# liangfu/dspnet

Measured on AMD Instinct MI355X. Metric: training images/sec at 512x512 multitask, higher is better.
Workload: dtype f32; 1 GPU; resnet-50 multitask (det+depth+seg) 512x512, 8 det classes, 19 seg classes, N=6132 anchors, forward+backward+SGD; batch_per_gpu=32, global_batch=32, parallelism=dp1, f16x2_fallback_calls=0

## Files before the change

### dspnet_amd/csrc/conv.hip

```cpp
#include "dspn_common.h"
#include "bn_final_job.h"
#include "dspn_store.h"
#include "dspn_pieces.h"
#include "conv_geom.h"
#include <cstdlib>
#include "../../include/dspn_nn.h"

using dspn::st_t;
using dspn::kHalf;
using dspn::u32x4_t;

namespace {

using dspn::conv::f32x16;
using dspn::conv::bf16x8;
using dspn::pieces::bf16x4;
typedef __attribute__((address_space(3))) bf16x4 lds_bf16x4;

constexpr int kLdsRowH = kHalf ? 72 : 40;
__device__ __forceinline__ bf16x4 to_bf16x4(const float4 v) {
  bf16x4 r = {(__bf16)v.x, (__bf16)v.y, (__bf16)v.z, (__bf16)v.w};
  return r;
}

// ... 1579 lines not shown
  if (cfg64 >= 0 && Cout > 32 && Cout <= 64 && tiles(kNtBm[cfg64], kNtBn[cfg64]) >= min_tiles) cfg = cfg64;
  if ((g_debug_bits >> 8) & 7) cfg = ((g_debug_bits >> 8) & 7) - 1;
  return cfg;
}
int output_absmax_pass(const st_t *out, const ConvGeom &g, hipStream_t s) {
#ifndef DSPN_HALF
  if (g.bn_dy_absmax && !g.bn_sums) {
    if (!(g.dense && g.obs == (long long)g.Hg * g.Wg * g.ldc && g.ldc % 4 == 0))
      return dspn::fail(DSPN_ERR_ARG_, "conv2d_forward: the output magnitude block needs a dense output with ldc %% 4 == 0");
    return dspn_absmax_f32(out, (long long)g.N * g.Hg * g.Wg, g.ldc, nullptr, nullptr, 0, reinterpret_cast<float *>(g.bn_dy_absmax), s);
  }
#endif
  return 0;
}
int dispatch_nt(const st_t *in, const st_t *w, const float *bias, st_t *out, const ConvGeom &g_in,
                hipStream_t s, SplitWs ws, const st_t *residual = nullptr) {
  ConvGeom g = g_in;
  g.dbg = g_debug_bits;
  constexpr uintptr_t amask = 4 * sizeof(st_t) - 1;
  if (g.ldc % 4 == 0 && g.obs % 4 == 0 && (reinterpret_cast<uintptr_t>(out) & amask) == 0 &&
      (!residual || (reinterpret_cast<uintptr_t>(residual) & amask) == 0))
    g.flags |= 16;
  {
    const long long ib = (long long)sizeof(st_t) * g.N * g.Hin * g.Win * g.Cin,
                    wb = (long long)sizeof(st_t) * g.Cout * g.WTAPS * g.Cin;
    if (ib >= (1ll << 31) || wb >= (1ll << 31))
      return dspn::fail(DSPN_ERR_ARG_, "conv: tensors of 2 GiB or more are not supported by the buffer-addressed kernel");
    g.in_bytes = (unsigned)ib; g.w_bytes = (unsigned)wb;
  }
  const long long M = (long long)g.N * g.Hg * g.Wg;
  if (M <= 0) return output_absmax_pass(out, g, s);
  const bool pre = !kHalf && g.bf16 >= 2 && ((g.Cin / kEPC) & 7) == 0;
  if (pre) {
    if (!g.w_planes)
      return dspn::fail(DSPN_ERR_ARG_, "conv: the split math modes with a multiple of 32 input channels (%d) need the weight operand as piece planes (dspn_conv2d_weight_planes_f32)", g.Cin);
    w = static_cast<const st_t *>(g.w_planes);
    g.w_bytes = (unsigned)((g.bf16 == 3 ? 4ll : 6ll) * g.Cout * g.WTAPS * g.Cin);
  }
  const int cfg = nt_config(M, g.Cout);
  const long long nblk = ((M + kNtBm[cfg] - 1) / kNtBm[cfg]) * ((g.Cout + kNtBn[cfg] - 1) / kNtBn[cfg]);
  const int nk = (g.TR * g.TS * (g.Cin / kEPC) + 7) >> 3;
  int splits = 1, per = nk;
  if (g.a_planes && !(pre && g.bf16 == 3 && !g.in_scale))
    return dspn::fail(DSPN_ERR_ARG_, "conv: a piece-plane operand needs DSPN_MATH_F32_F16X2, a multiple of 32 channels (%d) and no input affine", g.Cin);
  if (g.stats && (!g.dense || !(g.flags & 16) || g.Cout % 4 != 0))
    return dspn::fail(DSPN_ERR_ARG_, "conv2d_forward: output statistics need a dense, 16-byte aligned output with Cout %% 4 == 0");
  if (g.bn_sums && (g.in_scale || g.stats))
    return dspn::fail(DSPN_ERR_ARG_, "conv: BatchNorm-backward sums cannot be combined with an input affine or output statistics");
  if (g.bn_sums && (!(g.flags & 16) || g.Cout % 4 != 0))
    return dspn::fail(DSPN_ERR_ARG_, "conv2d_dgrad: BatchNorm sums need a 16-byte aligned dx with Cin %% 4 == 0");
  if (g.dense && nblk < 192 && nk >= 16 && ws.ptr && !g.stats && !g.bn_sums) {
    splits = (int)std::min<long long>((384 + nblk - 1) / nblk, nk / 8);
    splits = std::max(1, std::min(splits, 32));
    while (splits > 1 && sizeof(float) * (size_t)splits * M * g.Cout > ws.bytes) --splits;
    per = (nk + splits - 1) / splits;
    splits = (nk + per - 1) / per;
  }
  static const int eight_mode = (int)dspn::env_int("DSPN_NT_8WAVE", -1);
  const bool one_tap = g.TR * g.TS == 1;
  const bool eight = eight_mode == 0 ? false : eight_mode == 1 ? true : (kHalf || g.bf16 >= 2) ? true
                     : ((!g.stats && !g.bn_sums) || (eight_mode == 2 && one_tap && g.bn_sums) || (eight_mode == 3 && one_tap));
  bool wide_ok = splits == 1 && (cfg == 0 || (cfg == 2 && g.Cout > 32 && g.Cout <= 64)) && (g.flags & 16) && g.Cout % 4 == 0 &&
                 g.TR * g.TS > 0;
  if (kHalf) wide_ok = wide_ok && !g.in_scale && g.Cin % 64 == 0 && dspn::wide_tiles_mode() >= 2;
  else wide_ok = wide_ok && pre && g.bf16 == 3;
  if (const dspn::conv::WideRoute route = wide_ok ? dspn::conv::wide_route(g, M, nk) : dspn::conv::WideRoute{})
    return dspn::conv::launch_wide(route, in, w, bias, out, g, s, residual);
  const int rc = cfg == 0 && eight ? launch_nt<4, 2, 1, 2>(in, w, bias, out, g, s, splits, per, ws.ptr, residual)
                 : cfg == 0        ? launch_nt<2, 2, 2, 2>(in, w, bias, out, g, s, splits, per, ws.ptr, residual)
                 : cfg == 1        ? launch_nt<2, 2, 2, 1>(in, w, bias, out, g, s, splits, per, ws.ptr, residual)
                 : cfg == 2        ? launch_nt<2, 2, 1, 1>(in, w, bias, out, g, s, splits, per, ws.ptr, residual)
                                   : launch_nt<4, 1, 2, 1>(in, w, bias, out, g, s, splits, per, ws.ptr, residual);
  return rc ? rc : output_absmax_pass(out, g, s);
}

struct WgradPlan { int bm; int bn; int splits; int pps; };
constexpr int kPlanPK = 64;
static_assert(kPlanPK % kPK == 0, "split sizes must be whole k-steps");
long long wgrad_x_footprint(long long P, int Cin, int taps, int stride) { return taps > 1 ? 4ll * P * Cin * std::min(stride, 2) * std::min(stride, 2) : 0; }
WgradPlan wgrad_plan(long long P, int Cout, int J, long long x_bytes = 0, long long max_splits = 1 << 30) {
  WgradPlan p;
  p.bm = Cout <= 32 ? 32 : (Cout <= 64 ? 64 : 128);
  if (p.bm == 128 && (Cout + 63) / 64 * 64 < (Cout + 127) / 128 * 128) p.bm = 64;
  p.bn = (J <= 64 && p.bm == 128) ? 64 : 128;
  if (const char *e = getenv("DSPN_WG_TILE")) {
    const int t = atoi(e);
    p.bm = t == 0 ? 32 : (t == 1 ? 64 : 128);
    p.bn = t == 2 ? 64 : 128;
  }
  const long long tiles = (long long)((Cout + p.bm - 1) / p.bm) * ((J + p.bn - 1) / p.bn);
  const long long lds = 4ll * std::max(2 * kPK * (p.bm + p.bn), p.bm * (p.bn + 4));
  const long long slots = 256 * std::min<long long>(8, (160ll << 10) / lds);
  long long s_min = 1;
  if (x_bytes > 0) s_min = (x_bytes + (32ll << 20) - 1) / (32ll << 20);
  const long long s_max = std::max<long long>(1, std::min<long long>(std::min<long long>(P / 128, 1024), max_splits));
  s_min = std::min(s_min, s_max);
  const double flop_per_pix = 2.0 * p.bm * p.bn, slot_rate = 120e12 / (double)slots, ovh_pix = 160;
  double best = 1e30;
  long long splits = s_min;
  for (long long sp = s_min; sp <= s_max; ++sp) {
    const long long pps = ((P + sp - 1) / sp + kPlanPK - 1) / kPlanPK * kPlanPK;
    const long long real = (P + pps - 1) / pps;
    const long long rounds = (tiles * real + slots - 1) / slots;
    const double t = (double)rounds * ((double)pps + ovh_pix) * flop_per_pix / slot_rate +
                     (double)real * Cout * J * 8.0 / 4e12;
    if (t < best * 0.999) { best = t; splits = sp; }
    if (tiles * sp > 8 * slots) break;
  }
  if (const char *e = getenv("DSPN_WG_SPLITS")) splits = std::max<long long>(1, std::min<long long>(atoll(e), s_max));
  splits = std::min(splits, s_max);
  long long pps = ((P + splits - 1) / splits + kPlanPK - 1) / kPlanPK * kPlanPK;
  p.splits = (int)((P + pps - 1) / pps);
  p.pps = (int)pps;
  return p;
}

struct WgradLaunch { const st_t *x, *dy; float *slab; const WgradGeom &g; int kt, jt, rows; size_t lds; hipStream_t s; };
template <int WM, int WN, int TM, int TN, int MODE, bool INTF>
int launch_wgrad_impl(const WgradLaunch &a) {
  auto kern = conv_wgrad_kernel<WM, WN, TM, TN, MODE, INTF>;
  static dspn::KernelDeviceState st;
  if (const int dev = dspn::ensure_dynamic_lds(reinterpret_cast<const void *>(kern), a.lds, st, "conv_wgrad"); dev < 0) return dev;
  hipLaunchKernelGGL(kern, dim3(a.kt * a.jt, a.rows), dim3(WM * WN * 64), a.lds, a.s, a.x, a.dy, a.slab, a.g, a.kt, a.jt);
  return 0;
}
template <int WM, int WN, int TM, int TN, int MODE>
int launch_wgrad_mode(const WgradLaunch &a) {
  return a.g.in_scale ? launch_wgrad_impl<WM, WN, TM, TN, MODE, true>(a) : launch_wgrad_impl<WM, WN, TM, TN, MODE, false>(a);
}
template <int WM, int WN, int TM, int TN>
int launch_wgrad_tile(const WgradLaunch &a) {
  switch (kHalf ? 1 : a.g.bf16 != 3 ? a.g.bf16 : a.g.x_planes ? 5 + a.g.dy_planes : 3 + a.g.dy_planes) {
#ifndef DSPN_HALF
    case 6: return launch_wgrad_impl<WM, WN, TM, TN, 6, false>(a);
    case 5: return launch_wgrad_impl<WM, WN, TM, TN, 5, false>(a);
    case 4: return launch_wgrad_mode<WM, WN, TM, TN, 4>(a);
    case 3: return launch_wgrad_mode<WM, WN, TM, TN, 3>(a);
    case 2: return launch_wgrad_mode<WM, WN, TM, TN, 2>(a);
    case 0: return launch_wgrad_mode<WM, WN, TM, TN, 0>(a);
#endif
    default: return launch_wgrad_mode<WM, WN, TM, TN, 1>(a);
  }
}
static int launch_wgrad(int BM, int BN, const WgradLaunch &a) {
#ifndef DSPN_HALF
  static const bool wgw_env = dspn::env_int("DSPN_WGW", 1) != 0;
  if (a.g.bf16 == 3 && a.g.x_planes && a.g.dy_planes && BM == 128 && BN == 128 && wgw_env && dspn::wide_tiles_mode() != 1) {
    auto kern = conv_wgw_kernel<2, 2, 2>;
    const size_t lds_w = std::max<size_t>(2 * (size_t)kPK * (128 + 128) * 4, sizeof(float) * 128 * (128 + 4));
    static dspn::KernelDeviceState st;
    if (const int dev = dspn::ensure_dynamic_lds(reinterpret_cast<const void *>(kern), lds_w, st, "conv_wgrad (wide)"); dev < 0) return dev;
    hipLaunchKernelGGL(kern, dim3(a.kt * a.jt, a.rows), dim3(256), lds_w, a.s, a.x, a.dy, a.slab, a.g, a.kt, a.jt);
    return 0;
  }
#endif
  if (BM == 32) return launch_wgrad_tile<1, 4, 1, 1>(a);
  if (BM == 64) return launch_wgrad_tile<2, 2, 1, 2>(a);
  if (BN == 64) return launch_wgrad_tile<2, 2, 2, 1>(a);
  return launch_wgrad_tile<4, 2, 1, 2>(a);
}

}

extern "C" {

#ifdef DSPN_ABLATE
#ifdef DSPN_HALF
int dspn_debug_set_bf16(int bits) { g_debug_bits = bits; return 0; }
#else
int dspn_debug_set(int bits) { g_debug_bits = bits; return 0; }
int dspn_debug_read_stamps(unsigned *host, int words, int clear) {
  if (hipMemcpyFromSymbol(host, HIP_SYMBOL(g_phase_stamps), sizeof(unsigned) * (size_t)std::min(words, 8192 * 8)) != hipSuccess) return 1;
  if (clear) { static unsigned z[8192 * 8]; (void)hipMemcpyToSymbol(HIP_SYMBOL(g_phase_stamps), z, sizeof(z)); }
  return 0;
}
#endif
#endif

#ifndef DSPN_HALF
size_t dspn_conv2d_split_workspace_bytes(long long out_pixels, int Cout) {
  if (out_pixels <= 0 || Cout <= 0) return 0;
  const long long capped = std::min<long long>(out_pixels * Cout, 192ll * 64 * 64 * 4);
  return sizeof(float) * 32 * (size_t)capped;
}
#endif

static int split_math(int *math, int plane_bits) {
  const int flags = *math & (DSPN_MATH_UNSCALED_OK | plane_bits);
  *math &= ~flags;
  return flags;
}
static int check_math_mode(const char *who, int math) {
  DSPN_REQUIRE(math >= DSPN_MATH_FP32 && math <= DSPN_MATH_F32_F16X2, "%s: math is one of DSPN_MATH_*", who);
  return 0;
}
static int check_math_blocks(const char *who, int math, int flags, const float *a_absmax, const float *b_absmax) {
  DSPN_REQUIRE(dspn::kHalf || math != DSPN_MATH_F32_F16X2 || (flags & DSPN_MATH_UNSCALED_OK) || (a_absmax && b_absmax),
               "%s: DSPN_MATH_F32_F16X2 needs the magnitude block of both operands (dspn_absmax_f32); a caller who knows that every |operand| < 65504 passes math | DSPN_MATH_UNSCALED_OK", who);
  return 0;
}
struct InAffine { const float *scale, *shift; int relu; };
struct OpScales { const float *a, *b; int a_planes = 0; };

static int conv2d_forward_one(int math, OpScales scales, const st_t *x, InAffine tf, float *stats, float *minmax, const st_t *w, const void *w_planes, const float *bias, const st_t *residual, st_t *y, int N,
                            int H, int W, int Cin, int Cout, int R, int S, int stride, int pad_h, int pad_w,
                            int dil, int Ho, int Wo, long long y_batch_stride, int y_ldc,
                            int relu, int accumulate, void *workspace, size_t workspace_bytes,
                            void *stream) {
  DSPN_REQUIRE(x && (w || w_planes) && y, "conv2d_forward: null pointer");
  DSPN_REQUIRE(Cin % kEPC == 0, "conv2d_forward: Cin must be a multiple of %d (pad channels), got %d", kEPC, Cin);
  DSPN_REQUIRE(N > 0 && H > 0 && W > 0 && Cout > 0 && R > 0 && S > 0 && stride > 0 && dil > 0,
               "conv2d_forward: bad geometry");
  DSPN_REQUIRE(Ho == (H + 2 * pad_h - dil * (R - 1) - 1) / stride + 1 &&
                   Wo == (W + 2 * pad_w - dil * (S - 1) - 1) / stride + 1,
               "conv2d_forward: output size mismatch");
  ConvGeom g;
  memset(&g, 0, sizeof(g));
  g.N = N; g.Hin = H; g.Win = W; g.Cin = Cin; g.Hg = Ho; g.Wg = Wo;
  g.ish = stride; g.isw = stride; g.ioh = -pad_h; g.iow = -pad_w; g.idh = dil; g.idw = dil;
  g.TR = R; g.TS = S; g.WTAPS = R * S; g.WS = S; g.wr0 = 0; g.wrs = 1; g.ws0 = 0; g.wss = 1;
  g.Cout = Cout;
  g.ldc = y_ldc > 0 ? y_ldc : Cout;
  g.obs = y_batch_stride > 0 ? y_batch_stride : (long long)Ho * Wo * g.ldc;
  g.OW = Wo; g.osh = 1; g.osw = 1; g.ooh = 0; g.oow = 0;
  g.dense = (g.obs == (long long)Ho * Wo * g.ldc);
  g.flags = (bias ? 1 : 0) | (relu ? 2 : 0) | (accumulate ? 4 : 0) | (residual ? 8 : 0) | ((tf.scale && tf.relu) ? 32 : 0);
  g.in_scale = tf.scale; g.in_shift = tf.shift;
  g.stats = stats;
  g.minmax = (stats && !kHalf && math == DSPN_MATH_F32_F16X2) ? minmax : nullptr;
  g.bn_dy_absmax = (!stats && minmax && !kHalf && math == DSPN_MATH_F32_F16X2) ? reinterpret_cast<unsigned *>(minmax) : nullptr;
  g.bf16 = kHalf ? 1 : math;
  g.w_planes = w_planes;
  g.a_absmax = scales.a; g.b_absmax = scales.b;
  g.a_planes = scales.a_planes;
#ifndef DSPN_HALF
  if (math == DSPN_MATH_F32_F16X2 && R == 7 && S == 7 && stride == 2 && pad_h == 3 && pad_w == 3 && dil == 1 && Cin == 4 &&
      Cout == 64 && !bias && !relu && !accumulate && !residual && !tf.scale && g.dense && g.ldc == Cout && scales.a && scales.b &&
      !scales.a_planes && (reinterpret_cast<uintptr_t>(x) & 15) == 0 &&
      !g.bn_dy_absmax && (!stats || kNtBm[nt_config((long long)N * Ho * Wo, Cout)] == 64)) {
    const int rc = dspn::conv::launch_stem(x, w, y, N, H, W, Cin, Cout, Ho, Wo, scales.a, scales.b, stats, g.minmax, (hipStream_t)stream);
    if (rc <= 0) return rc;
  }
#endif
  return dispatch_nt(x, w, bias, y, g, (hipStream_t)stream,
                     SplitWs{static_cast<float *>(workspace), workspace ? workspace_bytes : 0}, residual);
}

static int batch_chunk(int N, long long bytes_per_image) {
  const long long lim = (1ll << 31) - 1;
  if (bytes_per_image <= 0 || N * bytes_per_image <= lim) return N;
  return (int)std::max<long long>(1, lim / bytes_per_image);
}

static int stats_layout(long long out_pixels, int Cout, int *tile_rows) {
  if (out_pixels <= 0 || Cout <= 0 || Cout % 4 != 0) return 0;
  const int bm = kNtBm[nt_config(out_pixels, Cout)];
  if (tile_rows) *tile_rows = bm;
  return (int)((out_pixels + bm - 1) / bm);
}
#ifndef DSPN_HALF
int dspn_conv2d_stats_layout(long long out_pixels, int Cout, int *tile_rows) { return stats_layout(out_pixels, Cout, tile_rows); }
#endif

int DSPN_FN(dspn_conv2d_forward_bn)(const st_t *x, const float *in_scale, const float *in_shift, int in_relu,
                               const st_t *w, const void *w_planes, const float *bias, const st_t *residual, st_t *y, int N,
                               int H, int W, int Cin, int Cout, int R, int S, int stride, int pad_h, int pad_w,
                               int dil, int Ho, int Wo, long long y_batch_stride, int y_ldc,
                               int relu, int accumulate, float *out_stats, size_t out_stats_bytes, float *out_minmax,
                               int math, const float *x_absmax, const float *w_absmax,
                               void *workspace, size_t workspace_bytes, void *stream) {
  DSPN_REQUIRE(N > 0 && H > 0 && W > 0 && Cin > 0, "conv2d_forward: bad geometry");
  const int flags = split_math(&math, DSPN_MATH_X_PLANES), x_planes = (flags & DSPN_MATH_X_PLANES) ? 1 : 0;
  if (const int rc = check_math_mode("conv2d_forward", math)) return rc;
  DSPN_REQUIRE(!x_planes || (!dspn::kHalf && math == DSPN_MATH_F32_F16X2 && Cin % 32 == 0 && x_absmax && !in_scale),
               "conv2d_forward: DSPN_MATH_X_PLANES needs DSPN_MATH_F32_F16X2, Cin %% 32 == 0, no input affine and the block the planes were cut by (x_absmax)");
  if (const int rc = check_math_blocks("conv2d_forward", math, flags, x_absmax, w_absmax)) return rc;
  DSPN_REQUIRE((in_scale == nullptr) == (in_shift == nullptr), "conv2d_forward: in_scale and in_shift go together");
  if (out_stats) {
    int tile_rows = 0;
    const int mt = stats_layout((long long)N * Ho * Wo, Cout, &tile_rows);
    DSPN_REQUIRE(mt > 0 && out_stats_bytes >= sizeof(float) * 2 * (size_t)mt * Cout,
                 "conv2d_forward: out_stats needs dspn_conv2d_stats_layout() tiles x 2 x Cout floats and Cout %% 4 == 0");
    DSPN_REQUIRE(batch_chunk(N, (long long)sizeof(st_t) * H * W * Cin) == N, "conv2d_forward: out_stats is not available for inputs of 2 GiB or more");
  }
  const int ldc = y_ldc > 0 ? y_ldc : Cout;
  const long long ybs = y_batch_stride > 0 ? y_batch_stride : (long long)Ho * Wo * ldc;
  const int nb = batch_chunk(N, (long long)sizeof(st_t) * H * W * Cin);
  for (int n0 = 0; n0 < N; n0 += nb) {
    const int n = std::min(nb, N - n0);
    const int rc = conv2d_forward_one(math, OpScales{x_absmax, w_absmax, x_planes}, x + (long long)n0 * H * W * Cin, InAffine{in_scale, in_shift, in_relu}, out_stats, out_minmax, w, w_planes, bias,
                                      residual ? residual + (long long)n0 * ybs : nullptr, y + (long long)n0 * ybs, n, H, W,
                                      Cin, Cout, R, S, stride, pad_h, pad_w, dil, Ho, Wo, y_batch_stride, y_ldc, relu,
                                      accumulate, workspace, workspace_bytes, stream);
    if (rc) return rc;
  }
  return 0;
}

#ifndef DSPN_HALF
int dspn_conv2d_forward_f32(const float *x, const float *w, const float *bias, const float *residual, float *y, int N,
                            int H, int W, int Cin, int Cout, int R, int S, int stride, int pad_h, int pad_w,
                            int dil, int Ho, int Wo, long long y_batch_stride, int y_ldc,
                            int relu, int accumulate, void *workspace, size_t workspace_bytes,
                            void *stream) {
  return dspn_conv2d_forward_bn_f32(x, nullptr, nullptr, 0, w, nullptr, bias, residual, y, N, H, W, Cin, Cout, R, S, stride, pad_h,
                                    pad_w, dil, Ho, Wo, y_batch_stride, y_ldc, relu, accumulate, nullptr, 0, nullptr,
// ... 380 lines not shown
```

### dspnet_amd/csrc/conv_geom.h

```cpp
#pragma once
#include <hip/hip_runtime.h>

namespace dspn {
namespace conv {

typedef float f32x16 __attribute__((ext_vector_type(16)));
typedef __bf16 bf16x8 __attribute__((ext_vector_type(8)));

template <typename st_t>
struct ConvGeomT {
  int N, Hin, Win, Cin;
  int Hg, Wg;
  int ish, isw, ioh, iow, idh, idw;
  int TR, TS;
  int WTAPS, WS, wr0, wrs, ws0, wss;
  int Cout;
  long long obs;
  int OW, osh, osw, ooh, oow, ldc;
  int flags;
  int dense;
  int dbg;
  int bf16;
  unsigned in_bytes, w_bytes;
  const float *in_scale, *in_shift;
  float *stats;
  float *minmax;
  const st_t *bn_x;
  const float *bn_scale, *bn_shift, *bn_mean, *bn_rstd;
  float *bn_sums;
  int bn_relu, bn_tile_base;
  unsigned *bn_dy_absmax;
  const float *a_absmax, *b_absmax;
  int a_planes;
  const void *w_planes;
};

__device__ __forceinline__ int xcd_remap(int bid, int nblk) {
  const int q = nblk >> 3, r = nblk & 7, x = bid & 7;
  const int start = x < r ? x * (q + 1) : r * (q + 1) + (x - r) * q;
  return start + (bid >> 3);
}


enum class WideTile { None, P256x128, P128x256, P128x128, P256x64, F128x256, F128x128, F256x64 };
enum class WideLoop { Plain, Spanning, Direct };
struct WideRoute {
  WideTile tile = WideTile::None; WideLoop loop = WideLoop::Plain;
  explicit operator bool() const { return tile != WideTile::None; }
};
WideRoute wide_route(const ConvGeomT<float> &g, long long M, int nk);
WideRoute wide_route(const ConvGeomT<__bf16> &g, long long M, int nk);
int launch_wide(WideRoute r, const float *in, const float *w_planes, const float *bias, float *out, const ConvGeomT<float> &g,
                hipStream_t s, const float *residual);
int launch_wide(WideRoute r, const __bf16 *in, const __bf16 *w, const float *bias, __bf16 *out, const ConvGeomT<__bf16> &g,
                hipStream_t s, const __bf16 *residual);

int launch_stem(const float *x, const float *w, float *y, int N, int H, int W, int Cin, int Cout, int Ho, int Wo,
                const float *x_absmax, const float *w_absmax, float *stats, float *minmax, hipStream_t s);

}
}
```

### dspnet_amd/csrc/conv_stem.h

```cpp

constexpr int kStemSeg = 256;
constexpr int kStemRing = 9;
constexpr int kStemRowPx = 2 * kStemSeg + 8;
constexpr int kStemRowBytes = kStemRowPx * 8;
constexpr int kStemWRow = 7 * 2 * 64 + 16;
constexpr int kStemWBytes = 64 * kStemWRow;

__global__ __launch_bounds__(512, 2) void conv_stem_f16x2_kernel(
    const float *__restrict__ x, const float *__restrict__ w, float *__restrict__ y, int N, int H, int W, int Ho, int Wo,
    int rows_per_strip, const float *__restrict__ x_absmax, const float *__restrict__ w_absmax,
    float *__restrict__ stats, float *__restrict__ minmax) {
  extern __shared__ __attribute__((aligned(1024))) char ssm[];
  char *sW = ssm;
  char *sX = ssm + kStemWBytes;
  float *sRed = reinterpret_cast<float *>(sX + kStemRing * 2 * kStemRowBytes);
  const int tid = threadIdx.x, lane = tid & 63, wave = tid >> 6;
  const float sc_a = operand_scale(x_absmax), sc_b = operand_scale(w_absmax);
  const float inv_a = 1.f / sc_a, inv_b = 1.f / sc_b;
  const int segs = Wo / kStemSeg, strips = (Ho + rows_per_strip - 1) / rows_per_strip;
  int b = blockIdx.x;
  const int seg = b % segs; b /= segs;
  const int strip = b % strips;
  const int n = b / strips;
  const int oy0 = strip * rows_per_strip, oy1 = min(Ho, oy0 + rows_per_strip);
  const int ix0 = 2 * seg * kStemSeg - 3;

  for (int i = tid; i < 64 * 7 * 8; i += 512) {
    const int s = i & 7, r = (i >> 3) % 7, k = i / 56;
    float4 v = make_float4(0.f, 0.f, 0.f, 0.f);
    if (s < 7) v = *reinterpret_cast<const float4 *>(w + ((k * 7 + r) * 7 + s) * 4);
    bf16x4 p0, p1;
    split2h(v, sc_b, p0, p1);
    repair_inf(p0, p1);
    *reinterpret_cast<bf16x4 *>(sW + k * kStemWRow + (r * 2 + 0) * 64 + s * 8) = p0;
    *reinterpret_cast<bf16x4 *>(sW + k * kStemWRow + (r * 2 + 1) * 64 + s * 8) = p1;
  }
  const float4 *xin = reinterpret_cast<const float4 *>(x) + (long long)n * H * W;
  auto load_px = [&](const int iy, const int p) __attribute__((always_inline)) {
    const int ix = ix0 + p;
    float4 v = make_float4(0.f, 0.f, 0.f, 0.f);
    if (p < kStemRowPx && (unsigned)iy < (unsigned)H && (unsigned)ix < (unsigned)W) v = xin[(long long)iy * W + ix];
    return v;
  };
  auto store_px = [&](const int slot, const int p, const float4 v) __attribute__((always_inline)) {
    if (p >= kStemRowPx) return;
    bf16x4 p0, p1;
    split2h(v, sc_a, p0, p1);
    *reinterpret_cast<bf16x4 *>(sX + (slot * 2 + 0) * kStemRowBytes + p * 8) = p0;
    *reinterpret_cast<bf16x4 *>(sX + (slot * 2 + 1) * kStemRowBytes + p * 8) = p1;
  };
  const int iy_base = 2 * oy0 - 3;
  for (int j = 0; j < 7; ++j) {
    store_px(j, tid, load_px(iy_base + j, tid));
    store_px(j, tid + 512, load_px(iy_base + j, tid + 512));
  }
  __syncthreads();

  const int frow = lane & 31, half = lane >> 5;
  const int px = wave * 32 + frow;
  f32x16 acc[2];
  for (int oy = oy0; oy < oy1; ++oy) {
    const int j0 = ((oy - oy0) * 2) % kStemRing;
    const int iy_new = 2 * oy + 4;
    float4 n0 = load_px(iy_new, tid), n1 = load_px(iy_new, tid + 512), n2 = load_px(iy_new + 1, tid), n3 = load_px(iy_new + 1, tid + 512);
#pragma unroll
    for (int r = 0; r < 16; ++r) { acc[0][r] = 0.f; acc[1][r] = 0.f; }
#pragma unroll
    for (int r = 0; r < 7; ++r) {
      int slot = j0 + r; slot = slot >= kStemRing ? slot - kStemRing : slot;
      const char *xa = sX + slot * 2 * kStemRowBytes + (2 * px + 2 * half) * 8;
      const char *wb = sW + frow * kStemWRow + r * 128 + half * 16;
#pragma unroll
      for (int kk = 0; kk < 2; ++kk) {
        const bf16x8 a0 = *reinterpret_cast<const bf16x8 *>(xa + kk * 32), a1 = *reinterpret_cast<const bf16x8 *>(xa + kStemRowBytes + kk * 32);
        bf16x8 b0[2], b1[2];
#pragma unroll
        for (int j = 0; j < 2; ++j) {
          b0[j] = *reinterpret_cast<const bf16x8 *>(wb + j * (32 * kStemWRow) + kk * 32);
          b1[j] = *reinterpret_cast<const bf16x8 *>(wb + j * (32 * kStemWRow) + 64 + kk * 32);
        }
#pragma unroll
        for (int j = 0; j < 2; ++j) {
          acc[j] = __builtin_amdgcn_mfma_f32_32x32x16_f16(__builtin_bit_cast(f16x8, a1), __builtin_bit_cast(f16x8, b0[j]), acc[j], 0, 0, 0);
          acc[j] = __builtin_amdgcn_mfma_f32_32x32x16_f16(__builtin_bit_cast(f16x8, a0), __builtin_bit_cast(f16x8, b1[j]), acc[j], 0, 0, 0);
          acc[j] = __builtin_amdgcn_mfma_f32_32x32x16_f16(__builtin_bit_cast(f16x8, a0), __builtin_bit_cast(f16x8, b0[j]), acc[j], 0, 0, 0);
        }
      }
    }
    const long long m_row = ((long long)n * Ho + oy) * Wo + seg * kStemSeg + wave * 32;
    float s1[2], mn[2], mx[2];
#pragma unroll
    for (int j = 0; j < 2; ++j) {
      const int co = j * 32 + frow;
      s1[j] = 0.f; mn[j] = __builtin_huge_valf(); mx[j] = -__builtin_huge_valf();
#pragma unroll
      for (int q = 0; q < 16; ++q) {
        const float v = acc[j][q] * inv_a * inv_b;
        acc[j][q] = v;
        y[(m_row + (q & 3) + 8 * (q >> 2) + 4 * half) * 64 + co] = v;
        s1[j] += v; mn[j] = fminf(mn[j], v); mx[j] = fmaxf(mx[j], v);
      }
    }
    if (stats) {
#pragma unroll
      for (int j = 0; j < 2; ++j) {
        const float mean16 = s1[j] * (1.f / 16.f);
        float m2 = 0.f;
#pragma unroll
        for (int q = 0; q < 16; ++q) { const float d = acc[j][q] - mean16; m2 += d * d; }
        const float mean_o = __shfl_xor(mean16, 32, 64), m2_o = __shfl_xor(m2, 32, 64);
        const float d = mean_o - mean16;
        const float mean32 = mean16 + 0.5f * d;
        const float m2_32 = m2 + m2_o + d * d * 8.f;
        const float mn32 = fminf(mn[j], __shfl_xor(mn[j], 32, 64)), mx32 = fmaxf(mx[j], __shfl_xor(mx[j], 32, 64));
        if (half == 0) *reinterpret_cast<float4 *>(sRed + (wave * 64 + j * 32 + frow) * 4) = make_float4(mean32, m2_32, mn32, mx32);
      }
    }
    __syncthreads();
    if (stats && tid < 256) {
      const int tl = tid >> 6, co = tid & 63;
      const float4 a = *reinterpret_cast<const float4 *>(sRed + ((2 * tl) * 64 + co) * 4);
      const float4 c = *reinterpret_cast<const float4 *>(sRed + ((2 * tl + 1) * 64 + co) * 4);
      const float d = c.x - a.x;
      const long long t = (((long long)n * Ho + oy) * Wo + seg * kStemSeg) / 64 + tl;
      stats[(t * 2 + 0) * 64 + co] = a.x + 0.5f * d;
      stats[(t * 2 + 1) * 64 + co] = a.y + c.y + d * d * 16.f;
      if (minmax) {
        minmax[(t * 2 + 0) * 64 + co] = fminf(a.z, c.z);
        minmax[(t * 2 + 1) * 64 + co] = fmaxf(a.w, c.w);
      }
    }
    int sl0 = j0 + 7; sl0 = sl0 >= kStemRing ? sl0 - kStemRing : sl0;
    int sl1 = j0 + 8; sl1 = sl1 >= kStemRing ? sl1 - kStemRing : sl1;
    store_px(sl0, tid, n0); store_px(sl0, tid + 512, n1);
    store_px(sl1, tid, n2); store_px(sl1, tid + 512, n3);
    __syncthreads();
  }
}

int launch_conv_stem(const float *x, const float *w, float *y, int N, int H, int W, int Cin, int Cout, int Ho, int Wo,
                     const float *x_absmax, const float *w_absmax, float *stats, float *minmax, hipStream_t s) {
  if (dspn::wide_tiles_mode() == 1) return 1;
  if (Cin != 4 || Cout != 64 || Wo % kStemSeg != 0 || Ho != (H + 6 - 7) / 2 + 1 || Wo != (W + 6 - 7) / 2 + 1) return 1;
  const int lds = kStemWBytes + kStemRing * 2 * kStemRowBytes + 8 * 64 * 4 * (int)sizeof(float);
  static dspn::KernelDeviceState st;
  if (const int dev = dspn::ensure_dynamic_lds(reinterpret_cast<const void *>(conv_stem_f16x2_kernel), (size_t)lds, st, "conv_stem"); dev < 0) return dev;
  int rows = 16;
  while (rows > 8 && (long long)N * ((Ho + rows - 1) / rows) * (Wo / kStemSeg) < 512) rows -= 4;
  const long long grid = (long long)N * ((Ho + rows - 1) / rows) * (Wo / kStemSeg);
  {
    dspn::ProfScope prof(0, s);
    hipLaunchKernelGGL(conv_stem_f16x2_kernel, dim3((unsigned)grid), dim3(512), lds, s, x, w, y, N, H, W, Ho, Wo, rows, x_absmax,
                       w_absmax, stats, minmax);
  }
  return dspn::check_launch("conv_stem");
}
```

### dspnet_amd/csrc/conv_wide.hip

```cpp
#include "dspn_common.h"
#include "dspn_store.h"
#include "dspn_pieces.h"
#include "conv_geom.h"
#include "../../include/dspn_nn.h"
#include <algorithm>
#include <type_traits>

namespace {
using namespace dspn::pieces;
using dspn::st_t;
using dspn::kHalf;
using dspn::u32x4_t;
using dspn::conv::f32x16;
using dspn::conv::bf16x8;
using dspn::conv::xcd_remap;
using dspn::conv::WideLoop;
using ConvGeom = dspn::conv::ConvGeomT<st_t>;
#include "conv_wide.h"
#ifndef DSPN_HALF
#include "conv_stem.h"
#endif
}

#ifndef DSPN_HALF
namespace {
struct AbsminRowsDesc { const float *w; unsigned *out; int rows, row_len; long long begin; };
__global__ __launch_bounds__(256) void absmin_rows_batch_kernel(const AbsminRowsDesc *__restrict__ d, int n) {
  __shared__ float sm[4];
  const long long row = blockIdx.x;
  int lo = 0, hi = n - 1;
  while (lo < hi) {
    const int mid = (lo + hi + 1) >> 1;
    if (d[mid].begin <= row) lo = mid; else hi = mid - 1;
  }
  const AbsminRowsDesc e = d[lo];
  const float *p = e.w + (row - e.begin) * (long long)e.row_len;
  float m = 0.f;
  for (int i = threadIdx.x; i < e.row_len; i += 256) m = fmaxf(m, fabsf(p[i]));
#pragma unroll
  for (int o = 32; o >= 1; o >>= 1) m = fmaxf(m, __shfl_xor(m, o, 64));
  if ((threadIdx.x & 63) == 0) sm[threadIdx.x >> 6] = m;
  __syncthreads();
  if (threadIdx.x == 0) {
    m = fmaxf(fmaxf(sm[0], sm[1]), fmaxf(sm[2], sm[3]));
    if (m > 0.f && m < __builtin_huge_valf()) atomicMin(e.out, __float_as_uint(m));
  }
}
__global__ __launch_bounds__(256) void tile_minmax_kernel(const float4 *__restrict__ x, long long rows, int C4, int tile_rows,
                                                          float4 *__restrict__ minmax) {
  const long long t = blockIdx.x;
  const long long r0 = t * tile_rows, r1 = r0 + tile_rows < rows ? r0 + tile_rows : rows;
  for (int c = blockIdx.y * 256 + threadIdx.x; c < C4; c += gridDim.y * 256) {
    constexpr float kInf = __builtin_huge_valf();
    float4 mn = make_float4(kInf, kInf, kInf, kInf), mx = make_float4(-kInf, -kInf, -kInf, -kInf);
    for (long long r = r0; r < r1; ++r) {
      const float4 v = x[r * C4 + c];
      mn.x = fminf(mn.x, v.x); mn.y = fminf(mn.y, v.y); mn.z = fminf(mn.z, v.z); mn.w = fminf(mn.w, v.w);
      mx.x = fmaxf(mx.x, v.x); mx.y = fmaxf(mx.y, v.y); mx.z = fmaxf(mx.z, v.z); mx.w = fmaxf(mx.w, v.w);
    }
    minmax[(t * 2 + 0) * C4 + c] = mn;
    minmax[(t * 2 + 1) * C4 + c] = mx;
  }
}
}

extern "C" {
int dspn_absmin_rows_batch_f32(const void *table, int n, long long total_rows, void *stream) {
  DSPN_REQUIRE(table && n > 0 && total_rows > 0 && total_rows < (1ll << 31), "absmin_rows_batch: bad argument");
  static_assert(sizeof(AbsminRowsDesc) == 32, "table row layout: 2 pointers, 2 ints, 1 int64");
  hipLaunchKernelGGL(absmin_rows_batch_kernel, dim3((unsigned)total_rows), dim3(256), 0, (hipStream_t)stream,
                     static_cast<const AbsminRowsDesc *>(table), n);
  return dspn::check_launch("absmin_rows_batch");
}
int dspn_tile_minmax_f32(const float *x, long long rows, int C, int tile_rows, float *minmax, void *stream) {
  DSPN_REQUIRE(x && minmax && rows > 0 && C > 0 && C % 4 == 0 && tile_rows > 0, "tile_minmax: bad argument (C must be a multiple of 4)");
  const long long tiles = (rows + tile_rows - 1) / tile_rows;
  DSPN_REQUIRE(tiles < (1ll << 31), "tile_minmax: too many tiles");
  hipLaunchKernelGGL(tile_minmax_kernel, dim3((unsigned)tiles, (C / 4 + 255) / 256), dim3(256), 0, (hipStream_t)stream,
                     reinterpret_cast<const float4 *>(x), rows, C / 4, tile_rows, reinterpret_cast<float4 *>(minmax));
  return dspn::check_launch("tile_minmax");
}
}

#endif

namespace dspn {
namespace conv {
#ifndef DSPN_HALF
int launch_stem(const float *x, const float *w, float *y, int N, int H, int W, int Cin, int Cout, int Ho, int Wo,
                const float *x_absmax, const float *w_absmax, float *stats, float *minmax, hipStream_t s) {
  return launch_conv_stem(x, w, y, N, H, W, Cin, Cout, Ho, Wo, x_absmax, w_absmax, stats, minmax, s);
}
#endif
static WideTile wide_tile_choice(long long M, int Cout, int nk, int fused_epilogue) {
  constexpr WideTile forced[5] = {WideTile::None, WideTile::None, WideTile::P256x128, WideTile::P128x256, WideTile::P128x128};
  const int mode = dspn::wide_tiles_mode();
  if (mode == 1) return WideTile::None;
  if (mode >= 2) return Cout <= 64 ? WideTile::P256x64 : forced[mode];
  if (Cout <= 64) return nk >= 4 ? WideTile::P256x64 : WideTile::None;
  if (nk < 4 && !(fused_epilogue && nk >= 2)) return WideTile::None;
  if (Cout % 256 == 0 && nk >= 8 && ((M + 127) / 128) * (Cout / 256) >= 256) return WideTile::P128x256;
  return WideTile::P128x128;
}
WideRoute wide_route(const ConvGeomT<st_t> &g, long long M, int nk) {
  WideRoute r{wide_tile_choice(M, g.Cout, nk, (g.stats || g.bn_sums) ? 1 : 0)};
#ifndef DSPN_HALF
  if (!r) return r;
  if (!g.a_planes)
    r.tile = r.tile == WideTile::P128x256 ? WideTile::F128x256 : r.tile == WideTile::P256x64 ? WideTile::F256x64 : WideTile::F128x128;
  const int xt = dspn::tile_spanning();
  const int bm = (r.tile == WideTile::P256x64 || r.tile == WideTile::F256x64) ? 256 : 128;
  const bool output_ok = g.dense && (g.flags & 16) && M % bm == 0 && M * g.ldc * (long long)sizeof(st_t) < (1ll << 31);
  if (xt == 0 || !output_ok) return r;
  if (r.tile == WideTile::P128x128) {
    if (nk >= 2) r.loop = WideLoop::Spanning;
  } else if (r.tile == WideTile::P128x256) {
    static const bool wide8 = dspn::env_int("DSPN_XT8", 1) != 0;
    if (nk >= 3 && wide8) r.loop = WideLoop::Spanning;
  } else if (bm == 256) {
    static const bool c64 = dspn::env_int("DSPN_XT64", 1) != 0;
    if (nk >= 2 && c64) r.loop = r.tile == WideTile::P256x64 ? WideLoop::Spanning : WideLoop::Direct;
  } else if (r.tile == WideTile::F128x128 && xt >= 2 && nk >= 2 && nk <= 8 && nk % 2 == 0 &&
             ((M + 127) / 128) * ((g.Cout + 127) / 128) >= 2048) {
    r.loop = WideLoop::Spanning;
  } else if (r.tile == WideTile::F128x128) {
    static const bool direct = dspn::env_int("DSPN_NTV_DIRECT", 1) != 0;
    if (nk >= 2 && direct) r.loop = WideLoop::Direct;
  } else if (r.tile == WideTile::F128x256) {
    static const bool direct8 = dspn::env_int("DSPN_NTV_DIRECT8", 1) != 0;
    if (nk >= 2 && direct8) r.loop = WideLoop::Direct;
  }
#endif
  return r;
}
int launch_wide(WideRoute r, const st_t *in, const st_t *w_planes, const float *bias, st_t *out, const ConvGeomT<st_t> &g,
                hipStream_t s, const st_t *residual) {
  switch (r.tile) {
    case WideTile::P256x128: return launch_ntw<4, 2, 3>(r.loop, in, w_planes, bias, out, g, s, residual);
    case WideTile::P128x256: return launch_ntw<2, 4, 3, 128, !kHalf>(r.loop, in, w_planes, bias, out, g, s, residual);
    case WideTile::P128x128: return launch_ntw<2, 2, 2, 128, !kHalf>(r.loop, in, w_planes, bias, out, g, s, residual);
    case WideTile::P256x64: return launch_ntw<4, 1, 2, 64, !kHalf>(r.loop, in, w_planes, bias, out, g, s, residual);
#ifndef DSPN_HALF
    case WideTile::F128x256: return launch_ntv<2, 4>(r.loop, in, w_planes, bias, out, g, s, residual);
    case WideTile::F128x128: return launch_ntv<2, 2, 128, true>(r.loop, in, w_planes, bias, out, g, s, residual);
    case WideTile::F256x64: return launch_ntv<4, 1, 64>(r.loop, in, w_planes, bias, out, g, s, residual);
#endif
    default: return dspn::fail(DSPN_ERR_ARG_, "conv: no wide tile shape %d", (int)r.tile);
  }
}
}
}
```

Measured before the change: 1005 images/s.

## Add specialized wgrad kernel for 7x7 stride-2 stem convolution

Adds a dedicated weight-gradient kernel for the 7x7/stride-2 stem conv with 4 input channels and 64 outputs. It stages dy and a row-run of input pixels in LDS as split f16 pairs, reuses the input run across the 7 filter rows per wave, and accumulates with MFMA using double buffering. The kernel also folds the BN-final job into extra grid rows. It replaces the generic tiled wgrad path, which handles the tiny Cin=4 stem poorly, at the cost of more specialized code guarded by many shape checks.

```diff
diff --git a/dspnet_amd/csrc/conv.hip b/dspnet_amd/csrc/conv.hip
--- a/dspnet_amd/csrc/conv.hip
+++ b/dspnet_amd/csrc/conv.hip
@@ -1755,6 +1755,16 @@
     if (const int dev = dspn::ensure_dynamic_lds(reinterpret_cast<const void *>(kern), lds_w, st, "conv_wgrad (wide)"); dev < 0) return dev;
     hipLaunchKernelGGL(kern, dim3(a.kt * a.jt, a.rows), dim3(256), lds_w, a.s, a.x, a.dy, a.slab, a.g, a.kt, a.jt);
     return 0;
+  }
+  const bool stem_env = dspn::env_int("DSPN_STEM_WGRAD", 1) != 0;
+  const WgradGeom &g = a.g;
+  if (g.bf16 == 3 && !g.x_planes && !g.dy_planes && !g.in_scale && g.dy_absmax && g.x_absmax && g.R == 7 && g.S == 7 && g.sh == 2 &&
+      g.sw == 2 && g.ph == 3 && g.pw == 3 && g.dh == 1 && g.dw == 1 && g.Cin == 4 && g.Cout == 64 && g.ldy >= 64 &&
+      g.Ho == (g.Hin - 1) / 2 + 1 && g.Wo == (g.Win - 1) / 2 + 1 && a.kt * a.jt == 2 &&
+      ((reinterpret_cast<uintptr_t>(a.x) | reinterpret_cast<uintptr_t>(a.dy)) & 15) == 0 && stem_env && dspn::wide_tiles_mode() != 1) {
+    const dspn::conv::StemWgradGeom sg{g.N, g.Hin, g.Win, g.Ho, g.Wo, g.ldy, g.pix_per_split, g.x_bytes, g.dy_bytes, g.dy_absmax, g.x_absmax,
+                                       g.job_rows, g.job};
+    return dspn::conv::launch_stem_wgrad(a.x, a.dy, a.slab, sg, a.rows, a.s);
   }
 #endif
   if (BM == 32) return launch_wgrad_tile<1, 4, 1, 1>(a);
diff --git a/dspnet_amd/csrc/conv_geom.h b/dspnet_amd/csrc/conv_geom.h
--- a/dspnet_amd/csrc/conv_geom.h
+++ b/dspnet_amd/csrc/conv_geom.h
@@ -1,5 +1,6 @@
 #pragma once
 #include <hip/hip_runtime.h>
+#include "bn_final_job.h"
 
 namespace dspn {
 namespace conv {
@@ -58,5 +59,14 @@
 int launch_stem(const float *x, const float *w, float *y, int N, int H, int W, int Cin, int Cout, int Ho, int Wo,
                 const float *x_absmax, const float *w_absmax, float *stats, float *minmax, hipStream_t s);
 
+struct StemWgradGeom {
+  int N, H, W, Ho, Wo, ldy, pix_per_split;
+  unsigned x_bytes, dy_bytes;
+  const float *dy_absmax, *x_absmax;
+  int job_rows;
+  dspn::BnFinalJob job;
+};
+int launch_stem_wgrad(const float *x, const float *dy, float *slab, const StemWgradGeom &g, int rows, hipStream_t s);
+
 }
 }
diff --git a/dspnet_amd/csrc/conv_stem.h b/dspnet_amd/csrc/conv_stem.h
--- a/dspnet_amd/csrc/conv_stem.h
+++ b/dspnet_amd/csrc/conv_stem.h
@@ -155,3 +155,144 @@
   }
   return dspn::check_launch("conv_stem");
 }
+
+constexpr int kSwgPK = 32;
+constexpr int kSwgRunPx = 2 * kSwgPK + 6;
+constexpr int kSwgXPlane = (kSwgRunPx + 2) * 8;
+constexpr int kSwgXBytes = 7 * 2 * kSwgXPlane;
+constexpr int kSwgARow = 64;
+constexpr int kSwgABytes = 2 * kSwgPK * kSwgARow;
+constexpr int kSwgStage = kSwgABytes + kSwgXBytes;
+
+typedef __attribute__((address_space(3))) bf16x4 swg_lds_bf16x4;
+
+__global__ __launch_bounds__(256, 2) void conv_stem_wgrad_f16x2_kernel(
+    const float *__restrict__ x, const float *__restrict__ dy, float *__restrict__ slab, const dspn::conv::StemWgradGeom g) {
+  extern __shared__ __attribute__((aligned(1024))) char ssm[];
+  if (g.job_rows > 0 && (int)blockIdx.y < g.job_rows) {
+    const int jb = (int)blockIdx.y * (int)gridDim.x + (int)blockIdx.x;
+    if (jb < g.job.blocks) dspn::bn_final_job_run(g.job, jb, ssm);
+    return;
+  }
+  const int grid_y = (int)gridDim.y - g.job_rows, block_y = (int)blockIdx.y - g.job_rows;
+  const int tid = threadIdx.x, lane = tid & 63, wave = tid >> 6;
+  const int lin = xcd_remap(block_y * 2 + (int)blockIdx.x, 2 * grid_y);
+  const int split = lin >> 1, cb = lin & 1;
+  const int P = g.N * g.Ho * g.Wo;
+  const int p_begin = min(P, split * g.pix_per_split), p_end = min(P, p_begin + g.pix_per_split);
+  const float sc_a = operand_scale(g.dy_absmax), sc_b = operand_scale(g.x_absmax);
+  const float inv = (1.f / sc_a) * (1.f / sc_b);
+  const bool nf_a = operand_nonfinite(g.dy_absmax), nf_b = operand_nonfinite(g.x_absmax);
+  const __amdgpu_buffer_rsrc_t rsrc_x = __builtin_amdgcn_make_buffer_rsrc(const_cast<float *>(x), 0, g.x_bytes, 0x00020000);
+  const __amdgpu_buffer_rsrc_t rsrc_dy = __builtin_amdgcn_make_buffer_rsrc(const_cast<float *>(dy), 0, g.dy_bytes, 0x00020000);
+  constexpr unsigned kOOB = 0x80000000u;
+
+  const int a_row = tid >> 3, a_ch = tid & 7;
+  int x_r[2], x_px[2];
+#pragma unroll
+  for (int i = 0; i < 2; ++i) { const int sl = tid + 256 * i; x_r[i] = sl / kSwgRunPx; x_px[i] = sl - x_r[i] * kSwgRunPx; }
+  int p = p_begin, pn, pho, pwo;
+  { const int hw = g.Ho * g.Wo; pn = p / hw; const int rem = p - pn * hw; pho = rem / g.Wo; pwo = rem - pho * g.Wo; }
+  float4 ra, rb[2];
+  auto ld4 = [](const __amdgpu_buffer_rsrc_t rs, const unsigned off) __attribute__((always_inline)) {
+    const auto t = __builtin_amdgcn_raw_buffer_load_b128(rs, (int)off, 0, 0);
+    return make_float4(__uint_as_float(t[0]), __uint_as_float(t[1]), __uint_as_float(t[2]), __uint_as_float(t[3]));
+  };
+  auto load_chunk = [&]() __attribute__((always_inline)) {
+    const int cnt = p < p_end ? min(min(kSwgPK, g.Wo - pwo), p_end - p) : 0;
+    ra = ld4(rsrc_dy, ((unsigned)((p + a_row) * g.ldy + cb * 32 + a_ch * 4) * 4u) | (a_row < cnt ? 0u : kOOB));
+#pragma unroll
+    for (int i = 0; i < 2; ++i) {
+      const int iy = 2 * pho - 3 + x_r[i], ix = 2 * pwo - 3 + x_px[i];
+      const bool v = x_r[i] < 7 && x_px[i] < 2 * cnt + 5 && (unsigned)iy < (unsigned)g.H && (unsigned)ix < (unsigned)g.W;
+      rb[i] = ld4(rsrc_x, ((unsigned)((pn * g.H + iy) * g.W + ix) * 16u) | (v ? 0u : kOOB));
+    }
+    p += cnt; pwo += cnt;
+    if (pwo >= g.Wo) { pwo = 0; if (++pho >= g.Ho) { pho = 0; ++pn; } }
+    return cnt;
+  };
+  auto store_chunk = [&](const int buf) __attribute__((always_inline)) {
+    char *sA = ssm + buf * kSwgStage, *sX = sA + kSwgABytes;
+    bf16x4 p0, p1;
+    split2h(ra, sc_a, p0, p1);
+    if (__builtin_expect(nf_a, 0)) repair_inf(p0, p1);
+    *reinterpret_cast<bf16x4 *>(sA + a_row * kSwgARow + a_ch * 8) = p0;
+    *reinterpret_cast<bf16x4 *>(sA + kSwgPK * kSwgARow + a_row * kSwgARow + a_ch * 8) = p1;
+#pragma unroll
+    for (int i = 0; i < 2; ++i) {
+      if (x_r[i] >= 7) continue;
+      split2h(rb[i], sc_b, p0, p1);
+      if (__builtin_expect(nf_b, 0)) repair_inf(p0, p1);
+      *reinterpret_cast<bf16x4 *>(sX + (x_r[i] * 2 + 0) * kSwgXPlane + x_px[i] * 8) = p0;
+      *reinterpret_cast<bf16x4 *>(sX + (x_r[i] * 2 + 1) * kSwgXPlane + x_px[i] * 8) = p1;
+    }
+  };
+
+  f32x16 acc[2];
+#pragma unroll
+  for (int q = 0; q < 16; ++q) { acc[0][q] = 0.f; acc[1][q] = 0.f; }
+  const int gl = lane >> 4, fq = (lane & 15) >> 2, fpp = lane & 3;
+  const int a_off = (8 * (gl >> 1) + fq) * kSwgARow + (16 * (gl & 1) + 4 * fpp) * 2;
+  const int b_off = (8 * (gl >> 1) + fq) * 16 + (16 * (gl & 1) + 4 * fpp) * 2;
+  auto frag = [](const char *base, const int row_bytes) __attribute__((always_inline)) {
+    const bf16x4 lo = __builtin_amdgcn_ds_read_tr16_b64_v4bf16((swg_lds_bf16x4 *)(base));
+    const bf16x4 hi = __builtin_amdgcn_ds_read_tr16_b64_v4bf16((swg_lds_bf16x4 *)(base + 4 * row_bytes));
+    const bf16x8 r = {lo[0], lo[1], lo[2], lo[3], hi[0], hi[1], hi[2], hi[3]};
+    return r;
+  };
+  const int r0 = 2 * wave, nr = wave < 3 ? 2 : 1;
+
+  int cnt = load_chunk();
+  store_chunk(0);
+  __syncthreads();
+  int buf = 0;
+  while (cnt > 0) {
+    const int cnt_next = load_chunk();
+    __builtin_amdgcn_sched_barrier(0);
+    const char *sA = ssm + buf * kSwgStage, *sX = sA + kSwgABytes;
+    const int nkk = cnt > 16 ? 2 : 1;
+    for (int kk = 0; kk < nkk; ++kk) {
+      const bf16x8 a0 = frag(sA + kk * 16 * kSwgARow + a_off, kSwgARow);
+      const bf16x8 a1 = frag(sA + kSwgPK * kSwgARow + kk * 16 * kSwgARow + a_off, kSwgARow);
+#pragma unroll
+      for (int u = 0; u < 2; ++u) {
+        if (u < nr) {
+          const char *xb = sX + (r0 + u) * 2 * kSwgXPlane + kk * 16 * 16 + b_off;
+          bf16x8 b0 = frag(xb, 16), b1 = frag(xb + kSwgXPlane, 16);
+          if (__builtin_expect(nf_b && cnt < kSwgPK, 0)) {
+#pragma unroll
+            for (int e = 0; e < 8; ++e)
+              if (kk * 16 + 8 * (lane >> 5) + e >= cnt) { b0[e] = (__bf16)0.f; b1[e] = (__bf16)0.f; }
+          }
+          acc[u] = __builtin_amdgcn_mfma_f32_32x32x16_f16(__builtin_bit_cast(f16x8, a1), __builtin_bit_cast(f16x8, b0), acc[u], 0, 0, 0);
+          acc[u] = __builtin_amdgcn_mfma_f32_32x32x16_f16(__builtin_bit_cast(f16x8, a0), __builtin_bit_cast(f16x8, b1), acc[u], 0, 0, 0);
+          acc[u] = __builtin_amdgcn_mfma_f32_32x32x16_f16(__builtin_bit_cast(f16x8, a0), __builtin_bit_cast(f16x8, b0), acc[u], 0, 0, 0);
+        }
+      }
+    }
+    store_chunk(buf ^ 1);
+    __syncthreads();
+    buf ^= 1;
+    cnt = cnt_next;
+  }
+  float *o = slab + ((long long)split * 64 + cb * 32) * 196;
+  const int col = lane & 31;
+  if (col < 28) {
+#pragma unroll
+    for (int u = 0; u < 2; ++u) {
+      if (u < nr) {
+#pragma unroll
+        for (int q = 0; q < 16; ++q)
+          o[((q & 3) + 8 * (q >> 2) + 4 * (lane >> 5)) * 196 + (r0 + u) * 28 + col] = acc[u][q] * inv;
+      }
+    }
+  }
+}
+
+int launch_conv_stem_wgrad(const float *x, const float *dy, float *slab, const dspn::conv::StemWgradGeom &g, int rows, hipStream_t s) {
+  const size_t lds = std::max<size_t>(2 * kSwgStage, 4096 + 4);
+  static dspn::KernelDeviceState st;
+  if (const int dev = dspn::ensure_dynamic_lds(reinterpret_cast<const void *>(conv_stem_wgrad_f16x2_kernel), lds, st, "conv_stem_wgrad"); dev < 0) return dev;
+  hipLaunchKernelGGL(conv_stem_wgrad_f16x2_kernel, dim3(2, (unsigned)rows), dim3(256), lds, s, x, dy, slab, g);
+  return 0;
+}
diff --git a/dspnet_amd/csrc/conv_wide.hip b/dspnet_amd/csrc/conv_wide.hip
--- a/dspnet_amd/csrc/conv_wide.hip
+++ b/dspnet_amd/csrc/conv_wide.hip
@@ -91,6 +91,9 @@
                 const float *x_absmax, const float *w_absmax, float *stats, float *minmax, hipStream_t s) {
   return launch_conv_stem(x, w, y, N, H, W, Cin, Cout, Ho, Wo, x_absmax, w_absmax, stats, minmax, s);
 }
+int launch_stem_wgrad(const float *x, const float *dy, float *slab, const StemWgradGeom &g, int rows, hipStream_t s) {
+  return launch_conv_stem_wgrad(x, dy, slab, g, rows, s);
+}
 #endif
 static WideTile wide_tile_choice(long long M, int Cout, int nk, int fused_epilogue) {
   constexpr WideTile forced[5] = {WideTile::None, WideTile::None, WideTile::P256x128, WideTile::P128x256, WideTile::P128x128};
```

Result: no change. 1005 images/s (-0.1%).
